# simeoncarstens/binf

Hardware: AMD Instinct MI355X
Metric: chain*leapfrog-steps/sec, 1024-d Gaussian (higher is better)
Workload: dtype f64

## Files before the change

### binf_amd/csrc/gauss_common.hpp

```cpp
#pragma once
#include "common.hpp"

namespace binf {

struct GaussNArgs {
    const double *q0;
    const double *p0;
    const double *u;
    double *q_out;
    double *samples;
    uint8_t *accepted;
    int64_t *n_accepted;
    double *e_before;
    double *e_after;
    double *dt_chain;
    double timestep;
    double k;
    double x0;
    double uprate;
    double downrate;
    int64_t C;
    int32_t D;
    int32_t nsteps;
    int32_t H;
    int32_t n;
    int32_t thin;
    int32_t n_adapt;
    uint64_t rng_seed;
    uint64_t rng_offset;
    int64_t chain_offset;
    double *p_dump;
    double *u_dump;
    double half_timestep;
    double c_lp;
};

inline void gauss_derived_args(GaussNArgs &a)
{
    a.half_timestep = 0.5 * a.timestep;
    a.c_lp = -0.5 * a.k;
}

struct GaussPlan {
    int32_t H;
    int LW;
    int tneed;
    bool regular;
    int64_t blocks;
};

inline GaussPlan gauss_plan(int64_t C, int64_t D)
{
    GaussPlan p;
    p.H = pairwise_tree_height(D);
    p.LW = p.H > 3 ? p.H - 3 : 0;
    p.tneed = 1;
    p.regular = true;
    int32_t len0 = -1;
    for (int g = 0; g < (1 << p.H); ++g) {
        Leaf L = pairwise_leaf((int32_t)D, p.H, g);
        int tn = (L.len + 7) / 8;
        if (tn > p.tneed) p.tneed = tn;
        if (len0 < 0) len0 = L.len;
        if (L.len != len0 || L.depth != p.H || (L.len & 7)) p.regular = false;
    }
    if (p.LW == 0) {
        const int64_t chains_per_wave = 64 >> (3 + p.H);
        const int64_t waves = (C + chains_per_wave - 1) / chains_per_wave;
        p.blocks = (waves + 3) / 4;
    } else {
        const int64_t chains_per_block = (p.LW == 3 ? 8 : 4) >> p.LW;
        p.blocks = (C + chains_per_block - 1) / chains_per_block;
    }
    return p;
}

int gauss_split_factor(int64_t C, int32_t H, bool regular, int tneed);
hipError_t launch_gauss_split(const GaussNArgs &a, int tneed, int split, bool unit, bool fma,
                              hipStream_t st);

struct LaneSum {
    double r;
    double tail;
};

template <bool REGULAR>
__device__ inline void lane_sum_add(LaneSum &s, double v, int t, int T)
{
    if (REGULAR) {
        s.r = (t == 0) ? v : s.r + v;
    } else {
        const double n = s.r + v;
        s.r = (t == 0) ? v : ((t < T) ? n : s.r);
        s.tail = (t == T) ? v : s.tail;
    }
}

__device__ inline void lane_sum_fused(LaneSum &s, double x, int t)
{
    s.r = (t == 0) ? x * x : __builtin_fma(x, x, s.r);
}

template <bool REGULAR, int LW = 0>
__device__ inline double chain_sum_finish(const LaneSum &s, int T, int rem,
                                          int lane, int H, int leafdepth,
                                          double *xch = nullptr, int wib = 0)
{
    const double r = sum8_f64(s.r);
    double res = r;
    if (!REGULAR) {
        res = (T > 0) ? r : -0.0;
        const int leafbase = lane & ~7;
#pragma unroll
        for (int i = 0; i < 7; ++i) {
            const double v = shfl_f64(s.tail, leafbase + i);
            const double n = res + v;
            res = (i < rem) ? n : res;
        }
    }
    const int hin = (LW > 0) ? 3 : H;
    for (int l = 0; l < hin; ++l) {
        const double o = xor_level_f64(res, l, lane);
        const double n = res + o;
        res = (leafdepth >= H - l) ? n : res;
    }
    if (LW > 0) {
#pragma unroll
        for (int l = 3; l < 3 + LW; ++l) {
            __syncthreads();
            if (lane == 0) xch[wib] = res;
            __syncthreads();
            const double o = xch[wib ^ (1 << (l - 3))];
            const double n = res + o;
            res = (leafdepth >= H - l) ? n : res;
        }
    }
    return 0.0 + res;
}

template <int H, int N>
__device__ inline void chain_sum_finish_fixed(double (&v)[N], int lane)
{
    static_assert(H >= 0 && H <= 3, "one-wave chains: at most 8 leaves");
#pragma unroll
    for (int i = 0; i < N; ++i) v[i] = v[i] + xor1_f64(v[i]);
#pragma unroll
    for (int i = 0; i < N; ++i) v[i] = v[i] + xor2_f64(v[i]);
#pragma unroll
    for (int i = 0; i < N; ++i) v[i] = v[i] + other_quad_f64(v[i]);
#pragma unroll
    for (int l = 0; l < H; ++l) {
#pragma unroll
        for (int i = 0; i < N; ++i) v[i] = v[i] + xor_level_f64(v[i], l, lane);
    }
#pragma unroll
    for (int i = 0; i < N; ++i) v[i] = 0.0 + v[i];
}

template <int CTRL, int BANKS_A>
__device__ inline double pair_level_f64(double a, double b)
{
    constexpr int BANKS_B = 0xf & ~BANKS_A;
    const int alo = __double2loint(a), ahi = __double2hiint(a);
    const int blo = __double2loint(b), bhi = __double2hiint(b);
    const int tlo = __builtin_amdgcn_update_dpp(alo, blo, CTRL, 0xf, BANKS_B, false);
    const int thi = __builtin_amdgcn_update_dpp(ahi, bhi, CTRL, 0xf, BANKS_B, false);
    const int ulo = __builtin_amdgcn_update_dpp(blo, alo, CTRL, 0xf, BANKS_A, false);
    const int uhi = __builtin_amdgcn_update_dpp(bhi, ahi, CTRL, 0xf, BANKS_A, false);
    return __hiloint2double(thi, tlo) + __hiloint2double(uhi, ulo);
}
__device__ inline double pair_xor4_f64(double a, double b) { return pair_level_f64<0x141, 0x5>(a, b); }
__device__ inline double pair_xor8_f64(double a, double b) { return pair_level_f64<0x128, 0x3>(a, b); }

__device__ inline double sum_xor16_f64(double v)
{
    const int lo = __double2loint(v), hi = __double2hiint(v);
    const auto a = __builtin_amdgcn_permlane16_swap(lo, lo, false, false);
    const auto b = __builtin_amdgcn_permlane16_swap(hi, hi, false, false);
    return __hiloint2double((int)b[0], (int)a[0]) + __hiloint2double((int)b[1], (int)a[1]);
}
__device__ inline double sum_xor32_f64(double v)
{
    const int lo = __double2loint(v), hi = __double2hiint(v);
    const auto a = __builtin_amdgcn_permlane32_swap(lo, lo, false, false);
    const auto b = __builtin_amdgcn_permlane32_swap(hi, hi, false, false);
    return __hiloint2double((int)b[0], (int)a[0]) + __hiloint2double((int)b[1], (int)a[1]);
}

template <int L>
__device__ inline double lane_value_f64(double v)
{
    return __hiloint2double(__builtin_amdgcn_readlane(__double2hiint(v), L),
                            __builtin_amdgcn_readlane(__double2loint(v), L));
}

__device__ inline double chain_sums_shared(double a, double b, double c, double d, bool four)
{
    a = a + xor1_f64(a);
    b = b + xor1_f64(b);
    c = c + xor1_f64(c);
    a = a + xor2_f64(a);
    b = b + xor2_f64(b);
    c = c + xor2_f64(c);
    if (four) {
        d = d + xor1_f64(d);
        d = d + xor2_f64(d);
        c = pair_xor4_f64(c, d);
    } else {
        c = c + other_quad_f64(c);
    }
    double r = pair_xor4_f64(a, b);
    r = pair_xor8_f64(r, c);
    r = sum_xor16_f64(r);
    r = sum_xor32_f64(r);
    return 0.0 + r;
}

__device__ inline double sgpr_const(unsigned long long bits)
{
    double c = __longlong_as_double((long long)bits);
    asm volatile("" : "+s"(c));
    return c;
}

__device__ inline double exp_clipped_range(double x)
{
    const double n = __builtin_rint(x * sgpr_const(0x3ff71547652b82feULL));
    double r = __builtin_fma(sgpr_const(0xbfe62e42fefa39efULL), n, x);
    r = __builtin_fma(sgpr_const(0xbc7abc9e3b39803fULL), n, r);
    double p = __builtin_fma(sgpr_const(0x3e5ade156a5dcb37ULL), r,
                             sgpr_const(0x3e928af3fca7ab0cULL));
    p = __builtin_fma(r, p, sgpr_const(0x3ec71dee623fde64ULL));
    p = __builtin_fma(r, p, sgpr_const(0x3efa01997c89e6b0ULL));
    p = __builtin_fma(r, p, sgpr_const(0x3f2a01a014761f6eULL));
    p = __builtin_fma(r, p, sgpr_const(0x3f56c16c1852b7b0ULL));
    p = __builtin_fma(r, p, sgpr_const(0x3f81111111122322ULL));
    p = __builtin_fma(r, p, sgpr_const(0x3fa55555555502a1ULL));
    p = __builtin_fma(r, p, sgpr_const(0x3fc5555555555511ULL));
    p = __builtin_fma(r, p, sgpr_const(0x3fe000000000000bULL));
    p = __builtin_fma(r, p, 1.0);
    p = __builtin_fma(r, p, 1.0);
    return __builtin_ldexp(p, (int)n);
}

template <bool BOUNDS = true>
__device__ inline bool metropolis_accept(double u, double x)
{
    if (!BOUNDS) {
        x = (x < -308.0) ? -308.0 : x;
        x = (x > 709.0) ? 709.0 : x;
        return u < exp_clipped_range(x);
    }
    const double margin = 0x1p-40;
    const double lo = (1.0 + x) - margin;
    const bool small = x >= -0.5 && x < 0.0;
    bool acc = (x >= 0.0 && u < 1.0) || (small && u < lo);
    if (!(acc || (small && u >= (1.0 + x + x * x * 0.5) + margin))) {
        x = (x < -308.0) ? -308.0 : x;
        x = (x > 709.0) ? 709.0 : x;
        acc = u < exp_clipped_range(x);
    }
    return acc;
}

enum { GAUSS_REJECT = 0, GAUSS_ACCEPT = 1, GAUSS_UNDECIDED = 2 };

__device__ inline int accept_decide(double u, double x, double delta)
{
    const double margin = 0x1p-40;
    const bool ok = (unsigned long long)__double_as_longlong(u) < 0x3ff0000000000000ULL &&
                    (unsigned long long)__double_as_longlong(delta) <= 0x3ea0000000000000ULL &&
                    __builtin_fabs(x) < __builtin_inf();
    const double xl = x - delta, xh = x + delta;
    const bool inb = xl >= -0.5;
    bool acc = inb && u < (1.0 + xl) - margin;
    bool rej = inb && xh < 0.0 && u >= (1.0 + xh + xh * xh * 0.5) + margin;
    if (ok && !(acc || rej)) {
        double c = (x < -308.0) ? -308.0 : x;
        c = (c > 709.0) ? 709.0 : c;
        const double y = exp_clipped_range(c);
        const double w = (delta + delta) * y;
        acc = u < (y - w) - margin;
        rej = u >= (y + w) + margin;
    }
    return (!ok || !(acc || rej)) ? GAUSS_UNDECIDED : (acc ? GAUSS_ACCEPT : GAUSS_REJECT);
}

__device__ inline double np_exp(double x)
{
    if (x > 709.782712893384) return __builtin_inf();
    if (x < -745.2) return 0.0;
    return exp_clipped_range(x);
}

template <bool UNIT>
__device__ inline double gauss_grad(double q, double k, double x0)
{
    return UNIT ? q : k * (q - x0);
}

template <bool FMA>
__device__ inline double kick(double p, double dt, double g)
{
    return FMA ? __builtin_fma(-dt, g, p) : p - dt * g;
}

template <bool FMA>
__device__ inline double drift(double q, double p, double dt)
{
    return FMA ? __builtin_fma(p, dt, q) : q + p * dt;
}

}
```

### binf_amd/csrc/hmc_gauss.hip

```cpp
#include "hmc_gauss_kernel.hpp"

namespace binf {

template <int TMAX, bool REGULAR, int LW, bool UDT = false, int HC = -1, bool FS = false>
static hipError_t launch_n_trl(const GaussNArgs &a, bool unit, bool fma, dim3 grid,
                               hipStream_t st)
{
    constexpr int BS = (LW == 3) ? 512 : 256;
    constexpr int R = GAUSS_RNG_HBM;
    constexpr bool FU = FS && gauss_fastsum_built(TMAX, HC, true);
    constexpr bool FN = FS && gauss_fastsum_built(TMAX, HC, false);
    if (unit) {
        if (fma) hmc_gauss_persist_kernel<TMAX, REGULAR, true, true, LW, R, UDT, HC, FU><<<grid, BS, 0, st>>>(a);
        else     hmc_gauss_persist_kernel<TMAX, REGULAR, true, false, LW, R, UDT, HC, FU><<<grid, BS, 0, st>>>(a);
    } else {
        if (fma) hmc_gauss_persist_kernel<TMAX, REGULAR, false, true, LW, R, UDT, HC, FN><<<grid, BS, 0, st>>>(a);
        else     hmc_gauss_persist_kernel<TMAX, REGULAR, false, false, LW, R, UDT, HC, FN><<<grid, BS, 0, st>>>(a);
    }
    return hipGetLastError();
}

static bool gauss_uniform_dt(const GaussNArgs &a)
{
    return a.dt_chain == nullptr && a.n_adapt == 0;
}

template <int TMAX, int HC>
static hipError_t launch_n_th(const GaussNArgs &a, bool unit, bool fma, dim3 grid,
                              hipStream_t st)
{
    if constexpr (HC == 3) {
        if (a.e_before == nullptr && a.e_after == nullptr) {
            if (gauss_uniform_dt(a))
                return launch_n_trl<TMAX, true, 0, true, HC, true>(a, unit, fma, grid, st);
            return launch_n_trl<TMAX, true, 0, false, HC, true>(a, unit, fma, grid, st);
        }
    }
    if (gauss_uniform_dt(a))
        return launch_n_trl<TMAX, true, 0, true, HC>(a, unit, fma, grid, st);
    return launch_n_trl<TMAX, true, 0, false, HC>(a, unit, fma, grid, st);
}

template <int TMAX>
static hipError_t launch_n_t(const GaussNArgs &a, bool regular, bool unit, bool fma,
                             dim3 grid, hipStream_t st)
{
    if (!regular)
        return launch_n_trl<TMAX, false, 0>(a, unit, fma, grid, st);
    if (a.H == 0) return launch_n_th<TMAX, 0>(a, unit, fma, grid, st);
    if constexpr (TMAX >= 12) {
        if (a.H == 1) return launch_n_th<TMAX, 1>(a, unit, fma, grid, st);
        if (a.H == 2) return launch_n_th<TMAX, 2>(a, unit, fma, grid, st);
        if (a.H == 3) return launch_n_th<TMAX, 3>(a, unit, fma, grid, st);
    }
    return hipErrorNotSupported;
}

template <int LW>
static hipError_t launch_n_wide(const GaussNArgs &a, bool regular, bool unit, bool fma,
                                dim3 grid, hipStream_t st)
{
    return regular ? launch_n_trl<16, true, LW>(a, unit, fma, grid, st)
                   : launch_n_trl<16, false, LW>(a, unit, fma, grid, st);
}

}

using namespace binf;

extern "C" int32_t binf_hmc_sample_n_gauss_f64(
    const double *q0, const double *p0, const double *u, double *q_out,
    double *samples, uint8_t *accepted, int64_t *n_accepted, double *e_before,
    double *e_after, double timestep, double *dt_chain, int64_t C, int64_t D,
    int32_t nsteps, int32_t n, int32_t thin, double k, double x0,
    int32_t n_adapt, double uprate, double downrate, int32_t mode, void *stream)
{
    if (C < 0 || D < 1 || nsteps < 1 || n < 1 || thin < 1 || n_adapt < 0)
        return fail(BINF_E_ARG, "hmc_sample_gauss: need C>=0, D>=1, nsteps>=1, n>=1, thin>=1, n_adapt>=0");
    if (mode != BINF_MODE_EXACT && mode != BINF_MODE_FMA)
        return fail(BINF_E_ARG, "hmc_sample_gauss: unknown mode %d", mode);
    if (C == 0) return 0;
    if (!q0 || !p0 || !u || !q_out)
        return fail(BINF_E_ARG, "hmc_sample_gauss: null buffer");
    if (n_adapt > 0 && !dt_chain)
        return fail(BINF_E_ARG, "hmc_sample_gauss: adaption needs dt_chain");
    if (D > 8192)
        return fail(BINF_E_UNSUPPORTED, "hmc_sample_gauss: D=%lld > 8192 not covered by the fused kernel", (long long)D);
    const GaussPlan plan = gauss_plan(C, D);
    const int32_t H = plan.H;
    if (H > 6)
        return fail(BINF_E_UNSUPPORTED, "hmc_sample_gauss: pairwise tree height %d > 6 for D=%lld", H, (long long)D);
    const int LW = plan.LW;
    const int64_t bytes = C * D * (int64_t)sizeof(double);
    const char *qo = (const char *)q_out, *qi = (const char *)q0, *pi = (const char *)p0;
    if ((qo != qi && qo < qi + bytes && qi < qo + bytes) ||
        (qo < pi + bytes * n && pi < qo + bytes))
        return fail(BINF_E_ALIAS, "hmc_sample_gauss: q_out overlaps q0/p0 (only q_out == q0 is allowed)");

    const int tneed = plan.tneed;
    const bool regular = plan.regular;
    GaussNArgs a;
    a.q0 = q0; a.p0 = p0; a.u = u; a.q_out = q_out; a.samples = samples;
    a.accepted = accepted; a.n_accepted = n_accepted; a.e_before = e_before;
    a.e_after = e_after; a.dt_chain = dt_chain; a.timestep = timestep; a.k = k;
    a.x0 = x0; a.uprate = uprate; a.downrate = downrate; a.C = C;
    a.D = (int32_t)D; a.nsteps = nsteps; a.H = H; a.n = n; a.thin = thin;
    a.n_adapt = n_adapt < n ? n_adapt : n;
    a.rng_seed = 0; a.rng_offset = 0; a.chain_offset = 0; a.p_dump = nullptr; a.u_dump = nullptr;
    gauss_derived_args(a);

    const int64_t blocks = plan.blocks;
    if (blocks > 0x7fffffffLL)
        return fail(BINF_E_UNSUPPORTED, "hmc_sample_gauss: too many chains");
    dim3 grid((unsigned)blocks);
    hipStream_t st = (hipStream_t)stream;
    const bool unit = (k == 1.0 && x0 == 0.0);
    const bool fma = (mode == BINF_MODE_FMA);
    hipError_t e;
    const int split = (LW == 0) ? gauss_split_factor(C, H, regular, tneed) : 1;
    if (split > 1)        e = launch_gauss_split(a, tneed, split, unit, fma, st);
    else if (LW == 1)     e = launch_n_wide<1>(a, regular && tneed == 16, unit, fma, grid, st);
    else if (LW == 2)     e = launch_n_wide<2>(a, regular && tneed == 16, unit, fma, grid, st);
    else if (LW == 3)     e = launch_n_wide<3>(a, regular && tneed == 16, unit, fma, grid, st);
    else if (tneed <= 1)  e = launch_n_t<1>(a, regular && tneed == 1, unit, fma, grid, st);
    else if (tneed <= 2)  e = launch_n_t<2>(a, regular && tneed == 2, unit, fma, grid, st);
    else if (tneed <= 4)  e = launch_n_t<4>(a, regular && tneed == 4, unit, fma, grid, st);
    else if (tneed <= 8)  e = launch_n_t<8>(a, regular && tneed == 8, unit, fma, grid, st);
    else if (tneed <= 12) e = launch_n_t<12>(a, regular && tneed == 12, unit, fma, grid, st);
    else                  e = launch_n_t<16>(a, regular && tneed == 16, unit, fma, grid, st);
    if (e != hipSuccess) return hip_fail(e, "hmc_gauss_persist_kernel launch");
    return 0;
}

extern "C" int32_t binf_hmc_gauss_waves_per_chain(int64_t C, int64_t D)
{
    if (C < 1 || D < 1 || D > 8192) return 0;
    const GaussPlan p = gauss_plan(C, D);
    if (p.H > 6) return 0;
    if (p.LW > 0) return 1 << p.LW;
    return gauss_split_factor(C, p.H, p.regular, p.tneed);
}

extern "C" int32_t binf_hmc_sample_gauss_f64(
    const double *q0, const double *p0, const double *u, double *q_out,
    uint8_t *accepted, int64_t *n_accepted, double *e_before, double *e_after,
    double timestep, double *dt_chain, int64_t C, int64_t D, int32_t nsteps,
    double k, double x0, int32_t adapt, double uprate, double downrate,
    int32_t mode, void *stream)
{
    if (C > 0 && D >= 1 && nsteps >= 1 && q0 && p0 && u && q_out && !accepted)
        return fail(BINF_E_ARG, "hmc_sample_gauss: null buffer");
    return binf_hmc_sample_n_gauss_f64(q0, p0, u, q_out, nullptr, accepted,
                                       n_accepted, e_before, e_after, timestep,
                                       dt_chain, C, D, nsteps, 1, 1, k, x0,
                                       adapt ? 1 : 0, uprate, downrate, mode,
                                       stream);
}
```

### binf_amd/csrc/hmc_gauss_kernel.hpp

```cpp
#pragma once
#include "gauss_common.hpp"
#include "xoshiro.hpp"

namespace binf {

enum { GAUSS_RNG_HBM = 0, GAUSS_RNG_FUSED = 1, GAUSS_RNG_DUMP = 2 };

constexpr int gauss_wpb(int LW, int RNG) { return (LW == 3 || RNG != GAUSS_RNG_HBM) ? 8 : 4; }

constexpr int GAUSS_STEP_UNROLL = 4;
constexpr int gauss_step_unroll(int TMAX, bool REGULAR, bool UNIT, bool FMA, int LW, int RNG)
{
    if (!REGULAR || LW != 0 || !UNIT) return 1;
    if ((TMAX == 12 && !FMA) || (TMAX == 4 && RNG == GAUSS_RNG_FUSED)) return 1;
    return GAUSS_STEP_UNROLL;
}

constexpr int GAUSS_PRIO_WINDOW = 4;
constexpr bool gauss_wave_priority(int LW, int RNG, int HC)
{
    return LW == 0 && RNG == GAUSS_RNG_HBM && HC == 3;
}

__device__ __forceinline__ void gauss_set_priority(int prio)
{
    switch (prio & 3) {
    case 0: __builtin_amdgcn_s_setprio(0); break;
    case 1: __builtin_amdgcn_s_setprio(1); break;
    case 2: __builtin_amdgcn_s_setprio(2); break;
    default: __builtin_amdgcn_s_setprio(3); break;
    }
}

constexpr int GAUSS_REDO_GS = 2;
template <int TMAX, int GS, bool UNIT, bool FMA>
__device__ inline bool gauss_exact_accept(const GaussNArgs &a, const double *qs, const double (*qs_lds)[64],
                                          int lane, const double *pc, double dt, double hdt, double c_lp,
                                          double u)
{
    LaneSum s0 = {0.0, 0.0}, spb = {0.0, 0.0}, sqa = {0.0, 0.0}, spa = {0.0, 0.0};
#pragma unroll 1
    for (int g = 0; g < TMAX / GS; ++g) {
        double qq[GS], pp[GS];
#pragma unroll
        for (int i = 0; i < GS; ++i) {
            const int t = g * GS + i;
            qq[i] = qs_lds ? qs_lds[t][lane] : qs[8 * t];
            pp[i] = pc[8 * t];
        }
#pragma unroll
        for (int i = 0; i < GS; ++i) {
            const int t = g * GS + i;
            const double d = UNIT ? qq[i] : qq[i] - a.x0;
            lane_sum_add<true>(s0, d * d, t, TMAX);
            lane_sum_add<true>(spb, pp[i] * pp[i], t, TMAX);
        }
#pragma unroll
        for (int i = 0; i < GS; ++i)
            pp[i] = kick<FMA>(pp[i], hdt, gauss_grad<UNIT>(qq[i], a.k, a.x0));
#pragma unroll 1
        for (int l = 0; l < a.nsteps - 1; ++l) {
#pragma unroll
            for (int i = 0; i < GS; ++i) {
                qq[i] = drift<FMA>(qq[i], pp[i], dt);
                pp[i] = kick<FMA>(pp[i], dt, gauss_grad<UNIT>(qq[i], a.k, a.x0));
            }
        }
#pragma unroll
        for (int i = 0; i < GS; ++i) {
            const int t = g * GS + i;
            qq[i] = drift<FMA>(qq[i], pp[i], dt);
            pp[i] = kick<FMA>(pp[i], hdt, gauss_grad<UNIT>(qq[i], a.k, a.x0));
            const double d = UNIT ? qq[i] : qq[i] - a.x0;
            lane_sum_add<true>(sqa, d * d, t, TMAX);
            lane_sum_add<true>(spa, pp[i] * pp[i], t, TMAX);
        }
    }
    const double r = chain_sums_shared(sqa.r, spa.r, spb.r, s0.r, true);
    const double Eb = -(c_lp * lane_value_f64<12>(r)) + 0.5 * lane_value_f64<8>(r);
    const double Ea = -(c_lp * lane_value_f64<0>(r)) + 0.5 * lane_value_f64<4>(r);
    return metropolis_accept<true>(u, -(Ea - Eb));
}

constexpr bool gauss_fastsum_built(int TMAX, int HC, bool UNIT) { return HC == 3 && (TMAX == 16 || !UNIT); }

template <int TMAX, bool REGULAR, bool UNIT, bool FMA, int LW, int RNG = GAUSS_RNG_HBM, bool UDT = false,
          int HC = -1, bool FASTSUM = false>
__global__ void __launch_bounds__(64 * gauss_wpb(LW, RNG))
hmc_gauss_persist_kernel(const GaussNArgs a)
{
    static_assert(HC < 0 || (REGULAR && LW == 0), "compile-time tree height: regular one-wave chains only");
    constexpr bool FIXED = HC >= 0;
    constexpr int HF = FIXED ? HC : 0;
    constexpr bool SHARED = HC == 3;
    static_assert(!FASTSUM || (SHARED && RNG == GAUSS_RNG_HBM), "fused sums: the shared-tree kernels, draws from HBM");
    constexpr bool EARLY = FIXED && UNIT && !SHARED;
    constexpr int WPB = gauss_wpb(LW, RNG);
    constexpr int WPC = 1 << LW;
    __shared__ double xch[WPB];
    __shared__ double ubc[WPB];
    constexpr int GS = (TMAX % 8 == 0) ? 8 : ((TMAX % 4 == 0) ? 4 : TMAX);
    constexpr int NG = TMAX / GS;
    constexpr int USTEP = gauss_step_unroll(TMAX, REGULAR, UNIT, FMA, LW, RNG);
    constexpr bool PRIO = gauss_wave_priority(LW, RNG, HC);
    __shared__ double stash[RNG == GAUSS_RNG_DUMP ? 1 : WPB][RNG == GAUSS_RNG_DUMP ? 1 : TMAX][64];
    __shared__ double zx[RNG == GAUSS_RNG_HBM ? 1 : XZIG_C + 1];
    if (RNG != GAUSS_RNG_HBM) {
        xzig_load_table(zx, threadIdx.x, WPB * 64);
        __syncthreads();
    }

    const int lane = threadIdx.x & 63;
    const int wib = threadIdx.x >> 6;
    const int64_t wave = (int64_t)blockIdx.x * WPB + wib;
    const int H = FIXED ? HC : a.H;
    const int lg = (LW > 0) ? 6 : 3 + H;
    const int slot = lane & ((1 << lg) - 1);
    const int j = slot & 7;
    const int wchain = wib & (WPC - 1);
    const int grp = (LW > 0) ? ((wchain << 3) | (lane >> 3)) : (slot >> 3);
    const bool writer = (LW > 0) ? (wchain == 0 && lane == 0) : (slot == 0);

    int off, n, leafdepth, canonical;
    if (REGULAR) {
        n = 8 * TMAX;
        off = grp * n;
        leafdepth = H;
        canonical = 1;
    } else {
        const Leaf L = pairwise_leaf(a.D, H, grp);
        off = L.off;
        n = L.len;
        leafdepth = L.depth;
        canonical = L.canonical;
    }
    const int T = (n >= 8) ? (n >> 3) : 0;
    const int rem = (n >= 8) ? (n & 7) : n;

    const int64_t raw = (LW > 0) ? (int64_t)blockIdx.x * (WPB / WPC) + (wib >> LW)
                                 : (wave << (6 - lg)) + (lane >> lg);
    const bool cvalid = raw < a.C;
    const int64_t chain = cvalid ? raw : a.C - 1;
    const int64_t CD = a.C * (int64_t)a.D;
    const int64_t base = chain * (int64_t)a.D + off + j;

    double dt = (UDT || !a.dt_chain) ? a.timestep : a.dt_chain[chain];
    double uu = 0.0;
    if (RNG == GAUSS_RNG_HBM) uu = a.u[chain];
    Xo128 gen = {0u, 0u, 0u, 0u};
    uint64_t gen_stream = 0;
    if (RNG != GAUSS_RNG_HBM) {
        const int cgrp = grp & ~((1 << (H - leafdepth)) - 1);
        gen_stream = (uint64_t)(chain + a.chain_offset) * (uint64_t)(8 << H) + (uint64_t)(cgrp * 8 + j);
    }
    __builtin_amdgcn_sched_barrier(0);

    double q[TMAX], pa[GS], pb[GS];
#pragma unroll
    for (int t = 0; t < GS; ++t) {
        const bool m = REGULAR || (8 * t + j < n);
        q[t] = (m && RNG != GAUSS_RNG_DUMP) ? a.q0[base + 8 * t] : 0.0;
    }
    if (RNG == GAUSS_RNG_HBM) {
#pragma unroll
        for (int i = 0; i < GS; ++i) {
            const bool m = REGULAR || (8 * i + j < n);
            pa[i] = m ? a.p0[base + 8 * i] : 0.0;
        }
    }
#pragma unroll
    for (int t = GS; t < TMAX; ++t) {
        const bool m = REGULAR || (8 * t + j < n);
        q[t] = (m && RNG != GAUSS_RNG_DUMP) ? a.q0[base + 8 * t] : 0.0;
    }

    const double c_lp = SHARED ? a.c_lp : -0.5 * a.k;
    LaneSum s0 = {0.0, 0.0};
    double Sq_state = 0.0;
    int64_t nacc = 0;

    const bool stash_lds = !(REGULAR && ((a.samples && a.thin == 1) || a.n == 1));
    double *rec = a.samples;
    const double *prev = a.q0;
    int rec_wait = a.thin;

    for (int s = 0; s < a.n; ++s) {
        if (PRIO) {
            const int left = (a.n - 1 - s) / GAUSS_PRIO_WINDOW;
            gauss_set_priority(left < 3 ? left : 3);
        }
        const double hdt = (UDT && SHARED) ? a.half_timestep : 0.5 * dt;
        if (RNG != GAUSS_RNG_HBM) gen = xo_seed(gen_stream, a.rng_seed, a.rng_offset + (uint64_t)s);
        if (RNG != GAUSS_RNG_DUMP && stash_lds) {
#pragma unroll
            for (int t = 0; t < TMAX; ++t) stash[wib][t][lane] = q[t];
        }

        const bool more = s + 1 < a.n;
        const double *pc = a.p0 + (int64_t)s * CD + base;
        const double *pn = more ? pc + CD : pc;
        double un = 0.0;
        if (RNG == GAUSS_RNG_HBM) un = a.u[(int64_t)(more ? s + 1 : s) * a.C + chain];

        LaneSum spb = {0.0, 0.0}, sqa = {0.0, 0.0}, spa = {0.0, 0.0};
        double Spb = 0.0;
#pragma unroll
        for (int g = 0; g < NG; ++g) {
            double(&cur)[GS] = (RNG == GAUSS_RNG_HBM && (g & 1)) ? pb : pa;
            double(&nxt)[GS] = (RNG == GAUSS_RNG_HBM && (g & 1)) ? pa : pb;
            if (RNG != GAUSS_RNG_HBM) {
                unsigned want = 0;
#pragma unroll
                for (int i = 0; i < GS; ++i)
                    if (REGULAR || (8 * (g * GS + i) + j < n)) want |= 1u << i;
                xzig_normals<GS>(cur, want, gen, zx);
                if (RNG == GAUSS_RNG_DUMP) {
                    if (cvalid && canonical) {
                        double *go = a.p_dump + (int64_t)s * CD + base;
#pragma unroll
                        for (int i = 0; i < GS; ++i)
                            if (want & (1u << i)) go[8 * (g * GS + i)] = cur[i];
                    }
                    continue;
                }
            } else if (g + 1 < NG) {
#pragma unroll
                for (int i = 0; i < GS; ++i) {
                    const int t = (g + 1) * GS + i;
                    const bool m = REGULAR || (8 * t + j < n);
                    nxt[i] = m ? pc[8 * t] : 0.0;
                }
            } else {
#pragma unroll
                for (int i = 0; i < GS; ++i) {
                    const bool m = REGULAR || (8 * i + j < n);
                    nxt[i] = m ? pn[8 * i] : 0.0;
                }
            }
            (void)nxt;
#pragma unroll
            for (int i = 0; i < GS; ++i)
                asm volatile("" : "+v"(cur[i]), "+v"(q[g * GS + i]));
            if (s == 0) {
#pragma unroll
                for (int i = 0; i < GS; ++i) {
                    const int t = g * GS + i;
                    const double d = UNIT ? q[t] : q[t] - a.x0;
                    if (FASTSUM) lane_sum_fused(s0, d, t);
                    else lane_sum_add<REGULAR>(s0, d * d, t, T);
                }
                if (FIXED && !SHARED && g == NG - 1) {
                    double v[1] = {s0.r};
                    chain_sum_finish_fixed<HF, 1>(v, lane);
                    Sq_state = v[0];
                }
            }
#pragma unroll
            for (int i = 0; i < GS; ++i) {
                if (FASTSUM) lane_sum_fused(spb, cur[i], g * GS + i);
                else lane_sum_add<REGULAR>(spb, cur[i] * cur[i], g * GS + i, T);
            }
            __builtin_amdgcn_sched_barrier(0);
            if (EARLY && g == NG - 1) {
                double v[1] = {spb.r};
                chain_sum_finish_fixed<HF, 1>(v, lane);
                Spb = v[0];
            }
#pragma unroll
            for (int i = 0; i < GS; ++i) {
                const int t = g * GS + i;
                cur[i] = kick<FMA>(cur[i], hdt, gauss_grad<UNIT>(q[t], a.k, a.x0));
            }
            if (EARLY && g == NG - 1) asm volatile("" : "+v"(Spb));
            if (USTEP == 1) {
                for (int l = 0; l < a.nsteps - 1; ++l) {
#pragma unroll
                    for (int i = 0; i < GS; ++i) {
                        const int t = g * GS + i;
                        q[t] = drift<FMA>(q[t], cur[i], dt);
                        cur[i] = kick<FMA>(cur[i], dt, gauss_grad<UNIT>(q[t], a.k, a.x0));
                    }
                }
            } else {
                const auto step = [&]() {
#pragma unroll
                    for (int i = 0; i < GS; ++i) {
                        const int t = g * GS + i;
                        q[t] = drift<FMA>(q[t], cur[i], dt);
                        cur[i] = kick<FMA>(cur[i], dt, gauss_grad<UNIT>(q[t], a.k, a.x0));
                    }
                };
                static_assert((USTEP & (USTEP - 1)) == 0, "the remainder below goes by the bits of its count");
                const int nl = a.nsteps > 1 ? a.nsteps - 1 : 0;
#pragma unroll 1
                for (int m = nl / USTEP; m > 0; --m) {
#pragma unroll
                    for (int k = 0; k < USTEP; ++k) step();
                }
#pragma unroll
                for (int b = USTEP >> 1; b > 0; b >>= 1) {
                    if (nl & b) {
#pragma unroll
                        for (int k = 0; k < b; ++k) step();
                    }
                }
            }
#pragma unroll
            for (int i = 0; i < GS; ++i) {
                const int t = g * GS + i;
                q[t] = drift<FMA>(q[t], cur[i], dt);
                cur[i] = kick<FMA>(cur[i], hdt, gauss_grad<UNIT>(q[t], a.k, a.x0));
            }
#pragma unroll
            for (int i = 0; i < GS; ++i) {
                const int t = g * GS + i;
                const double d = UNIT ? q[t] : q[t] - a.x0;
                if (FASTSUM) {
                    lane_sum_fused(sqa, d, t);
                    lane_sum_fused(spa, cur[i], t);
                } else {
                    lane_sum_add<REGULAR>(sqa, d * d, t, T);
                    lane_sum_add<REGULAR>(spa, cur[i] * cur[i], t, T);
                }
            }
            if (EARLY && g == NG - 1)
                asm volatile("" : "+v"(sqa.r), "+v"(spa.r));
            else
                asm volatile("" : "+v"(sqa.r), "+v"(spa.r), "+v"(spb.r));
            __builtin_amdgcn_sched_barrier(0);
        }
        if (RNG != GAUSS_RNG_HBM) {
            const double ud = xo_uniform53(gen);
            if (LW == 0) {
                uu = shfl_f64(ud, lane & ~((1 << lg) - 1));
            } else {
                if (wchain == 0 && lane == 0) ubc[wib] = ud;
                __syncthreads();
                uu = ubc[wib & ~(WPC - 1)];
                __syncthreads();
            }
            if (RNG == GAUSS_RNG_DUMP) {
                if (cvalid && writer) a.u_dump[(int64_t)s * a.C + chain] = uu;
                continue;
            }
        }
        if (RNG == GAUSS_RNG_HBM && (NG & 1)) {
#pragma unroll
            for (int i = 0; i < GS; ++i) pa[i] = pb[i];
        }
        double Sqa, Spa;
        if (SHARED) {
            const double r = chain_sums_shared(sqa.r, spa.r, spb.r, s0.r, s == 0);
            Sqa = lane_value_f64<0>(r);
            Spa = lane_value_f64<4>(r);
            Spb = lane_value_f64<8>(r);
            if (s == 0) Sq_state = lane_value_f64<12>(r);
        } else if (FIXED) {
            if (EARLY) {
                double v[2] = {sqa.r, spa.r};
                chain_sum_finish_fixed<HF, 2>(v, lane);
                Sqa = v[0];
                Spa = v[1];
            } else {
                double v[3] = {spb.r, sqa.r, spa.r};
                chain_sum_finish_fixed<HF, 3>(v, lane);
                Spb = v[0];
                Sqa = v[1];
                Spa = v[2];
            }
        } else {
            if (s == 0)
                Sq_state = chain_sum_finish<REGULAR, LW>(s0, T, rem, lane, H, leafdepth, xch, wib);
            Spb = chain_sum_finish<REGULAR, LW>(spb, T, rem, lane, H, leafdepth, xch, wib);
            Sqa = chain_sum_finish<REGULAR, LW>(sqa, T, rem, lane, H, leafdepth, xch, wib);
            Spa = chain_sum_finish<REGULAR, LW>(spa, T, rem, lane, H, leafdepth, xch, wib);
        }
        const double Eb = -(c_lp * Sq_state) + 0.5 * Spb;
        const double Ea = -(c_lp * Sqa) + 0.5 * Spa;

        bool acc;
        if (FASTSUM) {
            const int dec = accept_decide(uu, -(Ea - Eb), 0x1p-46 * (Eb + Ea));
            acc = dec == GAUSS_ACCEPT;
            if (__builtin_amdgcn_ballot_w64(dec == GAUSS_UNDECIDED || !(c_lp < 0.0)) != 0) {
                acc = gauss_exact_accept<TMAX, GAUSS_REDO_GS, UNIT, FMA>(
                    a, prev + base, stash_lds ? stash[wib] : nullptr, lane, pc, dt, hdt, c_lp, uu);
                __builtin_amdgcn_s_waitcnt(0);
            }
        } else {
            acc = metropolis_accept<SHARED>(uu, -(Ea - Eb));
        }

        if (!UDT && s < a.n_adapt)
            dt = acc ? dt * a.uprate : dt * a.downrate;
        if (cvalid && writer) {
            const int64_t o = (int64_t)s * a.C + chain;
            if (a.accepted) a.accepted[o] = acc ? 1 : 0;
            if (a.e_before) a.e_before[o] = Eb;
            if (a.e_after) a.e_after[o] = Ea;
        }
        if (acc) {
            Sq_state = Sqa;
            nacc += 1;
        } else {
            if (stash_lds) {
#pragma unroll
                for (int t = 0; t < TMAX; ++t) q[t] = stash[wib][t][lane];
            } else {
#pragma unroll
                for (int t = 0; t < TMAX; ++t) q[t] = prev[base + 8 * t];
            }
            __builtin_amdgcn_s_waitcnt(0);
        }
        if (a.samples && --rec_wait == 0) {
            rec_wait = a.thin;
            if (cvalid && canonical) {
                double *go = rec + base;
#pragma unroll
                for (int t = 0; t < TMAX; ++t)
                    if (REGULAR || (8 * t + j < n)) go[8 * t] = q[t];
            }
            prev = rec;
            rec += CD;
        }
        if (RNG == GAUSS_RNG_HBM) uu = un;
    }
    if (RNG == GAUSS_RNG_DUMP) return;
    if (PRIO) __builtin_amdgcn_s_setprio(0);

    if (cvalid && writer) {
        if (a.n_accepted) a.n_accepted[chain] += nacc;
        if (!UDT && a.n_adapt > 0 && a.dt_chain) a.dt_chain[chain] = dt;
    }
    if (cvalid && canonical) {
        double *go = a.q_out + base;
#pragma unroll
        for (int t = 0; t < TMAX; ++t)
            if (REGULAR || (8 * t + j < n)) go[8 * t] = q[t];
    }
}


}
```

Baseline: 5.482 billion.

## Derive Gaussian energy change from position sums, skipping final kick and momentum sum

Adds a ONESUM kernel variant for the unit Gaussian with uniform step size. It uses the closed-form leapfrog identity to estimate the Hamiltonian change from the change in sum(q^2) alone. That lets it drop the final half-kick and the per-step momentum-squared reduction, leaving a smaller cross-lane reduction. A widened error bound decides the accept/reject, and undecided cases fall back to the existing exact recomputation. It runs only when a domain check on timestep, k and nsteps passes, and it drops energy outputs for that path.

```diff
diff --git a/binf_amd/csrc/gauss_common.hpp b/binf_amd/csrc/gauss_common.hpp
--- a/binf_amd/csrc/gauss_common.hpp
+++ b/binf_amd/csrc/gauss_common.hpp
@@ -33,12 +33,27 @@
     double *u_dump;
     double half_timestep;
     double c_lp;
+    double c_dh;
+    double f_dh;
 };
+
+inline double gauss_onesum_factor(int32_t nsteps)
+{
+    return 0x1p-46 + (double)nsteps * 0x1p-48;
+}
+
+inline bool gauss_onesum_domain(const GaussNArgs &a)
+{
+    return a.timestep >= 0x1p-256 && a.k * a.timestep * a.timestep <= 1.0 && a.nsteps >= 1 &&
+           gauss_onesum_factor(a.nsteps) * 0x1p12 <= 0x1p-21;
+}
 
 inline void gauss_derived_args(GaussNArgs &a)
 {
     a.half_timestep = 0.5 * a.timestep;
     a.c_lp = -0.5 * a.k;
+    a.c_dh = ((a.k * a.timestep) * (a.k * a.timestep)) * 0.125;
+    a.f_dh = gauss_onesum_factor(a.nsteps);
 }
 
 struct GaussPlan {
@@ -211,6 +226,26 @@
     }
     double r = pair_xor4_f64(a, b);
     r = pair_xor8_f64(r, c);
+    r = sum_xor16_f64(r);
+    r = sum_xor32_f64(r);
+    return 0.0 + r;
+}
+
+__device__ inline double chain_sums_shared2(double a, double b, double d, bool three)
+{
+    a = a + xor1_f64(a);
+    b = b + xor1_f64(b);
+    a = a + xor2_f64(a);
+    b = b + xor2_f64(b);
+    double r = pair_xor4_f64(a, b);
+    if (three) {
+        d = d + xor1_f64(d);
+        d = d + xor2_f64(d);
+        d = d + other_quad_f64(d);
+        r = pair_xor8_f64(r, d);
+    } else {
+        r = r + xor8_f64(r);
+    }
     r = sum_xor16_f64(r);
     r = sum_xor32_f64(r);
     return 0.0 + r;
diff --git a/binf_amd/csrc/hmc_gauss.hip b/binf_amd/csrc/hmc_gauss.hip
--- a/binf_amd/csrc/hmc_gauss.hip
+++ b/binf_amd/csrc/hmc_gauss.hip
@@ -31,6 +31,14 @@
 {
     if constexpr (HC == 3) {
         if (a.e_before == nullptr && a.e_after == nullptr) {
+            if constexpr (TMAX == 16) {
+                if (unit && gauss_uniform_dt(a) && gauss_onesum_domain(a)) {
+                    constexpr int R = GAUSS_RNG_HBM;
+                    if (fma) hmc_gauss_persist_kernel<16, true, true, true, 0, R, true, 3, true, true><<<grid, 256, 0, st>>>(a);
+                    else     hmc_gauss_persist_kernel<16, true, true, false, 0, R, true, 3, true, true><<<grid, 256, 0, st>>>(a);
+                    return hipGetLastError();
+                }
+            }
             if (gauss_uniform_dt(a))
                 return launch_n_trl<TMAX, true, 0, true, HC, true>(a, unit, fma, grid, st);
             return launch_n_trl<TMAX, true, 0, false, HC, true>(a, unit, fma, grid, st);
diff --git a/binf_amd/csrc/hmc_gauss_kernel.hpp b/binf_amd/csrc/hmc_gauss_kernel.hpp
--- a/binf_amd/csrc/hmc_gauss_kernel.hpp
+++ b/binf_amd/csrc/hmc_gauss_kernel.hpp
@@ -85,7 +85,7 @@
 constexpr bool gauss_fastsum_built(int TMAX, int HC, bool UNIT) { return HC == 3 && (TMAX == 16 || !UNIT); }
 
 template <int TMAX, bool REGULAR, bool UNIT, bool FMA, int LW, int RNG = GAUSS_RNG_HBM, bool UDT = false,
-          int HC = -1, bool FASTSUM = false>
+          int HC = -1, bool FASTSUM = false, bool ONESUM = false>
 __global__ void __launch_bounds__(64 * gauss_wpb(LW, RNG))
 hmc_gauss_persist_kernel(const GaussNArgs a)
 {
@@ -94,6 +94,7 @@
     constexpr int HF = FIXED ? HC : 0;
     constexpr bool SHARED = HC == 3;
     static_assert(!FASTSUM || (SHARED && RNG == GAUSS_RNG_HBM), "fused sums: the shared-tree kernels, draws from HBM");
+    static_assert(!ONESUM || (FASTSUM && UNIT && UDT), "two sums: the unit Gaussian, one step size for the batch");
     constexpr bool EARLY = FIXED && UNIT && !SHARED;
     constexpr int WPB = gauss_wpb(LW, RNG);
     constexpr int WPC = 1 << LW;
@@ -309,13 +310,15 @@
             for (int i = 0; i < GS; ++i) {
                 const int t = g * GS + i;
                 q[t] = drift<FMA>(q[t], cur[i], dt);
-                cur[i] = kick<FMA>(cur[i], hdt, gauss_grad<UNIT>(q[t], a.k, a.x0));
+                if (!ONESUM) cur[i] = kick<FMA>(cur[i], hdt, gauss_grad<UNIT>(q[t], a.k, a.x0));
             }
 #pragma unroll
             for (int i = 0; i < GS; ++i) {
                 const int t = g * GS + i;
                 const double d = UNIT ? q[t] : q[t] - a.x0;
-                if (FASTSUM) {
+                if (ONESUM) {
+                    lane_sum_fused(sqa, d, t);
+                } else if (FASTSUM) {
                     lane_sum_fused(sqa, d, t);
                     lane_sum_fused(spa, cur[i], t);
                 } else {
@@ -323,7 +326,9 @@
                     lane_sum_add<REGULAR>(spa, cur[i] * cur[i], t, T);
                 }
             }
-            if (EARLY && g == NG - 1)
+            if (ONESUM)
+                asm volatile("" : "+v"(sqa.r), "+v"(spb.r));
+            else if (EARLY && g == NG - 1)
                 asm volatile("" : "+v"(sqa.r), "+v"(spa.r));
             else
                 asm volatile("" : "+v"(sqa.r), "+v"(spa.r), "+v"(spb.r));
@@ -348,8 +353,13 @@
 #pragma unroll
             for (int i = 0; i < GS; ++i) pa[i] = pb[i];
         }
-        double Sqa, Spa;
-        if (SHARED) {
+        double Sqa, Spa = 0.0;
+        if (ONESUM) {
+            const double r = chain_sums_shared2(sqa.r, spb.r, s0.r, s == 0);
+            Sqa = lane_value_f64<0>(r);
+            Spb = lane_value_f64<4>(r);
+            if (s == 0) Sq_state = lane_value_f64<8>(r);
+        } else if (SHARED) {
             const double r = chain_sums_shared(sqa.r, spa.r, spb.r, s0.r, s == 0);
             Sqa = lane_value_f64<0>(r);
             Spa = lane_value_f64<4>(r);
@@ -380,7 +390,9 @@
 
         bool acc;
         if (FASTSUM) {
-            const int dec = accept_decide(uu, -(Ea - Eb), 0x1p-46 * (Eb + Ea));
+            const double xt = ONESUM ? -(a.c_dh * (Sqa - Sq_state)) : -(Ea - Eb);
+            const double delta = ONESUM ? a.f_dh * ((Eb + Eb) + __builtin_fabs(xt)) : 0x1p-46 * (Eb + Ea);
+            const int dec = accept_decide(uu, xt, delta);
             acc = dec == GAUSS_ACCEPT;
             if (__builtin_amdgcn_ballot_w64(dec == GAUSS_UNDECIDED || !(c_lp < 0.0)) != 0) {
                 acc = gauss_exact_accept<TMAX, GAUSS_REDO_GS, UNIT, FMA>(
@@ -396,8 +408,10 @@
         if (cvalid && writer) {
             const int64_t o = (int64_t)s * a.C + chain;
             if (a.accepted) a.accepted[o] = acc ? 1 : 0;
-            if (a.e_before) a.e_before[o] = Eb;
-            if (a.e_after) a.e_after[o] = Ea;
+            if (!ONESUM) {
+                if (a.e_before) a.e_before[o] = Eb;
+                if (a.e_after) a.e_after[o] = Ea;
+            }
         }
         if (acc) {
             Sq_state = Sqa;
```

Measured after the change: 5.633 billion (median of 6 runs). 1.03x the previous value.
